# CodeKnight314/Goal-Conditioned-RL-Framework

Measured on AMD Instinct MI355X. Metric: gradient-steps/sec (HER sample + critic+actor update), higher is better.
Workload: dtype f32; 1 GPU; ddpg_pickplace_b256; agent=DDPG, batch_per_gpu=256, buffer_rows=1000000, state_dim=23, action_dim=4, hidden=256, layers=3, k_future=8, gradient_step=40, parallelism=single, hip_graph=True, rng=cpython-mt19937 (host) indices

## Files before the change

goal-conditioned-rl-framework_amd/csrc/agent_rowchain.inc:

```

struct PipeCtx {
  const StepCtrl* cur;
  const int* slot;
};


RowNet make_rownet(gcrl_agent* a, const NetSpec& n, const float* P, int which, int c = 0) {
  RowNet r;
  std::memset(&r, 0, sizeof(r));
  r.P = P;
  r.Wt = a->wt + a->wt_net[which] + (which >= 2 ? c * a->wt_cstride : 0);
  r.in = n.in_dim; r.jpad0 = round_up(n.in_dim, 4); r.H = n.H; r.L = n.L; r.out = n.out_dim;
  long long off = 0;
  for (int l = 0; l <= n.L; ++l) {
    r.w[l] = n.lin[l].w; r.b[l] = n.lin[l].b;
    if (l < n.L) { r.wt[l] = off; off += (long long)(l == 0 ? r.jpad0 : n.H) * n.H; }
  }
  return r;
}

int rc_rebuild_wt(gcrl_agent* a, hipStream_t st, bool targets_only = false) {
  auto one = [&](const RowNet& r) { return launch_wt_rebuild(st, r, const_cast<float*>(r.Wt)); };
  if (!targets_only && !a->sac) TRY(one(make_rownet(a, a->actor, a->P_actor(), 0)));
  if (a->has_target_actor) TRY(one(make_rownet(a, a->actor, a->P_tactor(), 1)));
  for (int c = 0; c < a->C; ++c) {
    if (!targets_only) TRY(one(make_rownet(a, a->critic, a->P_critic(c), 2, c)));
    TRY(one(make_rownet(a, a->critic, a->P_tcritic(c), 3, c)));
  }
  if (!targets_only) a->wt_dirty = false;
  return GCRL_OK;
}

int prof_drain(gcrl_agent* a) {
  if (a->prof_used == 0) return GCRL_OK;
  for (int i = 0; i < a->prof_used; ++i) {
    float ms = 0.f;
    GCRL_HIP(hipEventSynchronize(a->prof_b[i]));
    GCRL_HIP(hipEventElapsedTime(&ms, a->prof_a[i], a->prof_b[i]));
    a->prof_ms += ms;
  }
  std::vector<unsigned long long> clk(2 * (size_t)a->prof_used);
  GCRL_HIP(hipMemcpy(clk.data(), a->prof_clk, clk.size() * sizeof(unsigned long long), hipMemcpyDeviceToHost));
  for (int i = 0; i < a->prof_used; ++i)
    if (clk[2 * i + 1] > clk[2 * i]) a->prof_ticks += (double)(clk[2 * i + 1] - clk[2 * i]);
  a->prof_used = 0;
  return GCRL_OK;
}

bool heads_fold_on(const gcrl_agent* a) {
  return a->rowchain && a->cfg.kind == GCRL_AGENT_SAC && a->split_roles && a->slab_on() && !a->heads_fold_off && a->A <= 16 && a->bn_sync.world <= 1;
}

int rc_launch_chain(gcrl_agent* a, hipStream_t st, const PipeCtx& k, const PipeCtx& p, int what, const float* noise = nullptr) {
  RowChainArgs rc;
  std::memset(&rc, 0, sizeof(rc));
  rc.cur_k = k.cur; rc.cur_p = p.cur; rc.cb = a->ctrl();
  rc.actor = make_rownet(a, a->actor, a->P_actor(), 0);
  rc.tactor = make_rownet(a, a->actor, a->P_tactor(), 1);
  rc.C = a->C;
  for (int c = 0; c < a->C; ++c) {
    rc.critic[c] = make_rownet(a, a->critic, a->P_critic(c), 2, c);
    rc.tcritic[c] = make_rownet(a, a->critic, a->P_tcritic(c), 3, c);
  }
  const bool td3 = a->cfg.kind == GCRL_AGENT_TD3;
  rc.target_kind = a->sac ? TGT_MIN_ENT : (td3 ? TGT_MIN : TGT_DDPG);
  rc.loss_kind = td3 ? LOSS_SMOOTH_L1 : LOSS_MSE;
  if (a->sac) {
    rc.given_next = 1; rc.p_critic_only = 1;
    rc.logp_next = a->logp_next; rc.alpha = 0.2f;
    rc.pi = a->pi_buf;
  }
  rc.noise = noise; rc.policy_noise = (float)a->cfg.policy_noise; rc.noise_clamp = (float)a->cfg.noise_clamp;
  rc.seed = a->cfg.seed;
  rc.sa = a->sa; rc.nsa = a->nsa; rc.rbuf = a->rbuf; rc.dbuf = a->dbuf;
  rc.slot_x = a->slot_x; rc.slot_rd = a->slot_rd;
  rc.ldx = a->ldx; rc.ldl = a->row_ldl; rc.B = a->B; rc.S = a->S; rc.A = a->A; rc.Apad = a->Apad;
  const int nblk = (a->B + 4 * a->row_rg - 1) / (4 * a->row_rg);
  rc.linear_roles = 1;
  rc.nblk_k = (what & 1) ? nblk : 0;
  rc.nblk_p = (what & 2) ? nblk : 0;
  rc.hC = a->hC; rc.gC = a->rc_gC; rc.q = a->q; rc.y = a->ybuf; rc.dq = a->dq;
  rc.hA = a->hA; rc.gA = a->rc_gA; rc.hC2 = a->hC2; rc.q2 = a->q2; rc.dz = a->dact;
  rc.gamma = (float)a->cfg.gamma;
  rc.clamp_lo = (float)(-1.0 / (1.0 - a->cfg.gamma));
  rc.qt = a->qt;
  if (a->split_roles) {
    HeadsFold hfold;
    std::memset(&hfold, 0, sizeof(hfold));
    if (heads_fold_on(a)) {
      const NetSpec& an = a->actor;
      const long long BH = (long long)a->B * a->H;
      hfold.on = 1;
      hfold.P = a->P_actor();
      hfold.w_mean = an.lin[an.L].w; hfold.b_mean = an.lin[an.L].b; hfold.w_ls = an.lin[an.L + 1].w; hfold.b_ls = an.lin[an.L + 1].b;
      hfold.h_next = a->hN + (long long)((an.L - 1) & 1) * BH;
      hfold.h_cur = a->hA + (long long)(an.L - 1) * BH;
      hfold.eps_next = a->hf_eps_next; hfold.eps_cur = a->hf_eps_cur;
      hfold.logp_next = a->logp_next;
      hfold.pi = a->pi_buf; hfold.logp = a->logp; hfold.save_eps = a->epsbuf; hfold.save_std = a->stdbuf; hfold.head = a->headA;
      if (what & 1) {
        BnRunning& r = hfold.run;
        r.bstat[0] = a->bn_bstat; r.bstat[1] = a->hf_nf == 2 ? a->bn_bstat + (long long)an.L * 2 * a->H : nullptr;
        r.n = a->hf_nf; r.rmean = a->bn_rmean; r.rvar = a->bn_rvar; r.layers = an.L; r.H = a->H; r.B = a->B;
      }
    }
    static const bool cur_in_p = std::getenv("GCRL_HEADS_CUR_IN_P") != nullptr;
    hfold.cur_in_k = (hfold.on && a->hf_nf == 2 && !cur_in_p) ? 1 : 0;
    const HeadsFold* hfp = hfold.on ? &hfold : nullptr;
    const HeadsFold* hfp_p = (hfold.on && !hfold.cur_in_k) ? &hfold : nullptr;
    if (a->rc_merge) {
      rc.bar = reinterpret_cast<unsigned int*>(a->rc_bar); rc.status = a->status_dev;
      if (what & 1) TRY(launch_rowchain_split(st, rc, a->row_rg, 0, 3, hfp));
      if (what & 2) TRY(launch_rowchain_split(st, rc, a->row_rg, 1, 3, hfp_p));
      return GCRL_OK;
    }
    if (what & 1) { TRY(launch_rowchain_split(st, rc, a->row_rg, 0, 1, hfp)); TRY(launch_rowchain_split(st, rc, a->row_rg, 0, 2)); }
    if (what & 2) { TRY(launch_rowchain_split(st, rc, a->row_rg, 1, 1, hfp_p)); TRY(launch_rowchain_split(st, rc, a->row_rg, 1, 2)); }
    return GCRL_OK;
  }
  if (a->split_k) {
    if ((what & 1) && a->rc_merge_k) {
      rc.bar = reinterpret_cast<unsigned int*>(a->rc_bar); rc.status = a->status_dev; rc.producers_first = 1;
      TRY(launch_rowchain_split(st, rc, a->row_rg, 0, 3));
    } else if (what & 1) { TRY(launch_rowchain_split(st, rc, a->row_rg, 0, 1)); TRY(launch_rowchain_split(st, rc, a->row_rg, 0, 2)); }
    if (what & 2) { rc.nblk_k = 0; TRY(launch_rowchain_ddpg(st, rc, a->row_rg)); }
    return GCRL_OK;
  }
  if (a->ddpg_ksplit && (what & 1)) {
    rc.k_split = 1; rc.producers_first = 1;
    rc.bar = reinterpret_cast<unsigned int*>(a->rc_bar); rc.status = a->status_dev;
  }
  if (!a->prof || what != 3) return launch_rowchain_ddpg(st, rc, a->row_rg);
  if (a->prof_used == gcrl_agent::kProfPairs) TRY(prof_drain(a));
  const unsigned long long init[2] = {~0ull, 0ull};
  rc.clk = a->prof_clk + 2 * a->prof_used;
  GCRL_HIP(hipMemcpyAsync(rc.clk, init, sizeof(init), hipMemcpyHostToDevice, st));
  GCRL_HIP(hipEventRecord(a->prof_a[a->prof_used], st));
  TRY(launch_rowchain_ddpg(st, rc, a->row_rg));
  GCRL_HIP(hipEventRecord(a->prof_b[a->prof_used], st));
  a->prof_used++;
  a->prof_launches++;
  return GCRL_OK;
}

void rc_add_dw(gcrl_agent* a, Launches& ls, const PipeCtx& c, bool critic, bool fused) {
  const int B = a->B, L = a->L, H = a->H;
  const NetSpec& net = critic ? a->critic : a->actor;
  const long long BH = (long long)B * H;
  for (int k = 0; k < (critic ? a->C : 1); ++k) {
    float* Gp = critic ? a->G_critic(k) : a->G_actor();
    const float* hid = critic ? a->hC + (long long)k * L * BH : a->hA;
    const float* gr = critic ? a->rc_gC + (long long)k * L * BH : a->rc_gA;
    const float* x0 = a->sa;
    for (int l = L; l >= 0; --l) {
      const float* G = l == L ? (critic ? a->dq + (long long)k * B : a->dact) : gr + (long long)l * BH;
      const long long ldg = l == L ? (critic ? 1 : a->Apad) : H;
      GemmDesc dw = bwd_dw(G, ldg, l == 0 ? x0 : hid + (long long)(l - 1) * BH, l == 0 ? a->ldx : H, Gp, net.lin[l], B);
      if (l == 0) { dw.slot = c.slot; dw.b_slot = a->slot_x; }
      if (fused) dw.sumsq_out = critic ? a->parts_c + (long long)k * a->nparts_c + a->part_off_c[l] : a->parts_a + a->part_off_a[l];
      dw_split_form(a, dw, critic ? k : -1, l);
      ls.add(0, dw);
    }
  }
}

void rc_adam_extras(gcrl_agent* a, AdamArgs& ad, bool critic) {
  const NetSpec& net = critic ? a->critic : a->actor;
  ad.wt = a->wt + a->wt_net[critic ? 2 : 0];
  ad.wt_target = a->wt + a->wt_net[critic ? 3 : 1];
  ad.wt_net_stride = critic ? a->wt_cstride : 0;
  ad.n_seg = 0;
  int blk = 0;
  long long pos = 0, off = 0;
  auto flat = [&](long long beg, long long end) {
    if (end <= beg) return;
    AdamSeg& s = ad.seg[ad.n_seg++];
    s.beg = beg; s.dst = 0; s.rows = 1; s.cols = (int)(end - beg); s.tiled = 0; s.pad = 0;
    s.blk0 = blk; s.nblk = (int)((end - beg + 256 * kAdamPerThread - 1) / (256 * kAdamPerThread)); blk += s.nblk;
  };
  for (int l = 0; l < net.L; ++l) {
    const Lin& ln = net.lin[l];
    flat(pos, ln.w);
    AdamSeg& s = ad.seg[ad.n_seg++];
    s.beg = ln.w; s.dst = off; s.rows = ln.out; s.cols = ln.in; s.tiled = 1; s.pad = 0;
    s.blk0 = blk; s.nblk = ((ln.out + kAdamTile - 1) / kAdamTile) * ((ln.in + kAdamTile - 1) / kAdamTile); blk += s.nblk;
    pos = ln.w + (long long)ln.out * ln.in;
    off += (long long)(l == 0 ? round_up(net.in_dim, 4) : net.H) * net.H;
  }
  flat(pos, net.numel);
  ad.seg_blocks = blk;
  if (critic) {
    ad.td_q = a->q; ad.td_y = a->ybuf; ad.td_n = a->B; ad.td_C = a->C;
    ad.td_loss_kind = a->cfg.kind == GCRL_AGENT_TD3 ? LOSS_SMOOTH_L1 : LOSS_MSE;
  }
}

void of_fill_net(gcrl_agent* a, DwAdamNet& n, bool critic, int k, const StepCtrl* cur, bool polyak) {
  const int B = a->B, L = a->L, H = a->H;
  const NetSpec& net = critic ? a->critic : a->actor;
  const long long BH = (long long)B * H;
  std::memset(&n, 0, sizeof(n));
  float* Gp = critic ? a->G_critic(k) : a->G_actor();
  const float* hid = critic ? a->hC + (long long)k * L * BH : a->hA;
  const float* gr = critic ? a->rc_gC + (long long)k * L * BH : a->rc_gA;
  const std::vector<int>& poff = critic ? a->part_off_c : a->part_off_a;
  std::vector<long long> wt_off((size_t)L + 1, -1);
  long long off = 0;
  for (int l = 0; l < L; ++l) { wt_off[l] = off; off += (long long)(l == 0 ? round_up(net.in_dim, 4) : H) * H; }
  int q = 0;
  for (int l = L; l >= 0; --l, ++q) {
    const float* G = l == L ? (critic ? a->dq + (long long)k * B : a->dact) : gr + (long long)l * BH;
    const long long ldg = l == L ? (critic ? 1 : a->Apad) : H;
    GemmDesc dw = bwd_dw(G, ldg, l == 0 ? a->sa : hid + (long long)(l - 1) * BH, l == 0 ? a->ldx : H, Gp, net.lin[l], B);
    if (l == 0) { dw.slot = &cur->batch_slot; dw.b_slot = a->slot_x; }
    n.d[q] = dw;
    n.o.lay[q] = DwAdamLayer{net.lin[l].w, net.lin[l].b, wt_off[l], poff[l] / 4, 0};
  }
  n.o.nl = L + 1;
  n.o.cur = cur;
  n.o.which = critic ? 1 : 0;
  const long long go = critic ? a->goff_critic + (long long)k * a->critic_stride : a->goff_actor;
  n.o.p = critic ? a->P_critic(k) : a->P_actor();
  n.o.m = a->adam_m + go; n.o.v = a->adam_v + go;
  n.o.target = critic ? a->P_tcritic(k) : (polyak ? a->P_tactor() : nullptr);
  n.o.wt = a->wt + a->wt_net[critic ? 2 : 0] + (critic ? (long long)k * a->wt_cstride : 0);
  n.o.wt_target = a->wt + a->wt_net[critic ? 3 : 1] + (critic ? (long long)k * a->wt_cstride : 0);
  n.o.clip = (critic && k == 0 && a->cfg.kind == GCRL_AGENT_TD3) ? -1.f : (float)a->cfg.grad_clip;
  n.o.polyak = polyak ? 1 : 0;
  n.o.metric_index = critic ? MET_CRITIC_GRAD + k : MET_ACTOR_GRAD;
  const int ni = critic ? k : a->C;
  n.o.slots = reinterpret_cast<unsigned long long*>(a->of_slots) + (long long)ni * 2 * a->of_stride;
  n.o.slot_stride = (int)a->of_stride;
  n.o.seq = reinterpret_cast<unsigned int*>(a->of_seq) + ni * 32;
  if (critic) {
    if (k == 0) {
      n.o.td_q = a->q; n.o.td_y = a->ybuf; n.o.td_n = a->B; n.o.td_C = a->C;
      n.o.td_loss_kind = a->cfg.kind == GCRL_AGENT_TD3 ? LOSS_SMOOTH_L1 : LOSS_MSE;
    }
  } else {
    n.o.mean_x = a->q2; n.o.mean_n = a->B; n.o.mean_scale = -1.0f; n.o.mean_index = MET_ACTOR_LOSS;
  }
}

void of_common(gcrl_agent* a, DwAdamArgs& da) {
  std::memset(&da, 0, sizeof(da));
  da.beta2 = (float)kBeta2; da.w1 = (float)(1.0 - kBeta1); da.w2 = (float)(1.0 - kBeta2); da.eps = (float)kAdamEps;
  da.tau = (float)a->cfg.tau; da.one_m_tau = (float)(1.0 - a->cfg.tau);
  da.metrics = a->metrics_dev;
  da.status = a->status_dev;
  da.poll_first_sleep = 0; da.poll_sleep = 2; da.poll_gate = 0; da.leaders = 1;
}

bool of_phase_critics(const gcrl_agent* a, int variant) {
  return a->opt_fuse && a->cfg.kind != GCRL_AGENT_DDPG && (variant & V_FUSED_NORM) && !(variant & V_XCHG) && !(variant & V_WEIGHTS);
}
bool of_phase_actor(const gcrl_agent* a, int variant) { return of_phase_critics(a, variant) && !a->sac; }
int of_launch_critics(gcrl_agent* a, hipStream_t st, int variant) {
  DwAdamArgs da;
  of_common(a, da);
  for (int k = 0; k < a->C; ++k) of_fill_net(a, da.net[k], true, k, &a->ctrl()->cur_b, (variant & V_POLYAK_C) != 0);
  da.nnets = a->C;
  if ((variant & V_ADV) && !(variant & V_ACTOR)) da.advance = a->ctrl();
  return launch_dw_adam(st, da);
}
int of_launch_actor(gcrl_agent* a, hipStream_t st, int variant) {
  DwAdamArgs da;
  of_common(a, da);
  of_fill_net(a, da.net[0], false, 0, &a->ctrl()->cur_b, a->cfg.kind == GCRL_AGENT_TD3 && (variant & V_POLYAK_A) != 0);
  da.nnets = 1;
  if (variant & V_ADV) da.advance = a->ctrl();
  return launch_dw_adam(st, da);
}

int of_launch_ddpg(gcrl_agent* a, hipStream_t st, int what, bool adv, bool polyak) {
  DwAdamArgs da;
  of_common(a, da);
  int n = 0;
  if (what & 1) of_fill_net(a, da.net[n++], true, 0, &a->ctrl()->cur_b, polyak);
  if (what & 2) of_fill_net(a, da.net[n++], false, 0, what == 3 ? &a->ctrl()->prev_b : &a->ctrl()->cur_b, polyak);
  da.nnets = n;
  if (adv) da.advance = a->ctrl();
#ifdef GCRL_OF_STAMPS
  static unsigned long long* stamps = nullptr;
  static long long launches = 0;
  static const long long at = std::getenv("GCRL_OF_STAMPS_AT") ? std::atoll(std::getenv("GCRL_OF_STAMPS_AT")) : 3000;
  const char* path = std::getenv("GCRL_OF_STAMPS");
  if (path && !stamps) { GCRL_HIP(hipMalloc((void**)&stamps, 2 * 2048 * 8 * sizeof(unsigned long long))); }
  hipStreamCaptureStatus cs = hipStreamCaptureStatusNone;
  (void)hipStreamIsCapturing(st, &cs);
  const bool take = path && what == 3 && cs == hipStreamCaptureStatusNone && launches >= at && launches < at + 8;
  if (what == 3 && cs == hipStreamCaptureStatusNone) ++launches;
  da.stamps = take ? stamps : nullptr;
  if (take) {
    GCRL_HIP(hipMemsetAsync(stamps, 0, 2 * 2048 * 8 * sizeof(unsigned long long), st));
    TRY(launch_dw_adam(st, da));
    GCRL_HIP(hipStreamSynchronize(st));
    std::vector<unsigned long long> h(2 * 2048 * 8);
    GCRL_HIP(hipMemcpy(h.data(), stamps, h.size() * sizeof(unsigned long long), hipMemcpyDeviceToHost));
    FILE* f = std::fopen(path, launches - 1 == at ? "wb" : "ab");
    if (f) { std::fwrite(h.data(), sizeof(unsigned long long), h.size(), f); std::fclose(f); }
    return GCRL_OK;
  }
#endif
  return launch_dw_adam(st, da);
}
```

goal-conditioned-rl-framework_amd/csrc/dw_adam.h:

```cpp
#pragma once
#include "gemm_mfma.h"
#include "ops.h"

namespace gcrl {

struct DwAdamNet {
  DwAdamNetArgs o;
  GemmDesc d[kFusedMaxLayers];
};
struct DwAdamArgs {
  int nnets;
  float beta2, w1, w2, eps, tau, one_m_tau;
  float* metrics;
  CtrlBlock* advance;
  unsigned int* status;
  int leaders;
  int poll_gate;
  int poll_first_sleep, poll_sleep;
#ifdef GCRL_OF_STAMPS
  unsigned long long* stamps;
#endif
  DwAdamNet net[2];
};
int launch_dw_adam(hipStream_t st, DwAdamArgs& a);

}
```

goal-conditioned-rl-framework_amd/csrc/dw_adam.hip:

```cpp
#include "dw_adam.h"

#include <algorithm>

#include "adam_math.h"
#include "meet.h"
#include "pop.h"

namespace gcrl {
namespace {

constexpr unsigned long long kSlotEmpty = ~0ull;
constexpr int kLeaderMinTiles = 64;
static_assert(kFusedMaxLayers == 5, "DwNetHead::tile0 holds the first tiles of problems 1..4");

#ifdef GCRL_OF_STAMPS
#define OF_STAMP(k) of_t[k] = wall_clock64()
#else
#define OF_STAMP(k) do { } while (0)
#endif

template <class T>
__device__ __forceinline__ T load_uniform(const T* p) {
  static_assert(sizeof(T) % 4 == 0, "whole dwords");
  typedef const unsigned int __attribute__((address_space(4))) cu32;
  cu32* q = reinterpret_cast<cu32*>(reinterpret_cast<uintptr_t>(p));
  union { T v; unsigned int w[sizeof(T) / 4]; } u;
#pragma unroll
  for (unsigned i = 0; i < sizeof(T) / 4; ++i) u.w[i] = q[i];
  return u.v;
}

typedef float __attribute__((address_space(1))) gfloat;
typedef unsigned long long __attribute__((address_space(1))) gu64;
typedef unsigned int __attribute__((address_space(1))) gu32;

template <class T>
__device__ __forceinline__ void pin(T& v) {
  static_assert(sizeof(T) % 4 == 0, "whole dwords");
  unsigned int* w = reinterpret_cast<unsigned int*>(&v);
#pragma unroll
  for (unsigned i = 0; i < sizeof(T) / 4; ++i) asm volatile("" : "+s"(w[i]));
}

struct DwProb {
  const float* G; const float* X; float* dW; float* db;
  long long pw, pb, wt_dst;
  int ldg, ldx, out, in, K, tiles_n, slot0, x_slot;
};
struct DwNetHead {
  int ntiles, nl, which, slot_stride;
  int tile0[4];
  const StepCtrl* cur; unsigned int* seq; unsigned long long* slots;
  int polyak, grid_x;
};
struct DwNetPtrs {
  float *p, *m, *v, *target, *wt, *wt_target;
  float clip; int pad;
};
struct DwNetK {
  DwNetHead h;
  DwNetPtrs ptr;
  int metric_index, mean_n;
  const float* mean_x; float mean_scale; int mean_index;
  const float* td_q; const float* td_y; int td_n, td_C, td_loss_kind, pad;
  DwProb prob[kFusedMaxLayers];
};
struct DwAdamK {
  float beta2, w1, w2, eps, tau, one_m_tau;
  int leaders, poll_gate, poll_first_sleep, poll_sleep;
  float* metrics; CtrlBlock* advance; unsigned int* status;
#ifdef GCRL_OF_STAMPS
  unsigned long long* stamps;
#endif
  DwNetK net[2];
};

__global__ __launch_bounds__(256, 5) void dw_adam_kernel(DwAdamK a) {
  const unsigned bx = blockIdx.x, by = blockIdx.y;
#include "dw_adam_body.inc"
}

__global__ __launch_bounds__(256, 5) void dw_adam_pop_kernel(const DwAdamK* __restrict__ tab) {
  const DwAdamK& a = tab[blockIdx.z];
  const unsigned bx = blockIdx.x, by = blockIdx.y;
#include "dw_adam_body.inc"
}

}

long long dw_adam_capacity() { return meet_capacity((const void*)dw_adam_kernel, 256, 0); }

int launch_dw_adam(hipStream_t st, DwAdamArgs& a) {
  GCRL_CHECK_ARG(a.nnets >= 1 && a.nnets <= 2, "dw_adam: %d nets (1 or 2)", a.nnets);
  DwAdamK k;
  std::memset(&k, 0, sizeof(k));
  k.beta2 = a.beta2; k.w1 = a.w1; k.w2 = a.w2; k.eps = a.eps; k.tau = a.tau; k.one_m_tau = a.one_m_tau;
  k.leaders = a.leaders; k.poll_gate = a.poll_gate; k.poll_first_sleep = a.poll_first_sleep; k.poll_sleep = a.poll_sleep;
  k.metrics = a.metrics; k.advance = a.advance; k.status = a.status;
#ifdef GCRL_OF_STAMPS
  k.stamps = a.stamps;
#endif
  int widest = 0;
  for (int i = 0; i < a.nnets; ++i) {
    DwAdamNet& n = a.net[i];
    DwNetK& kn = k.net[i];
    GCRL_CHECK_ARG(n.o.nl >= 1 && n.o.nl <= kFusedMaxLayers && n.o.slots && n.o.seq && n.o.cur, "dw_adam: net %d: %d problems / missing slots", i, n.o.nl);
    int tiles = 0;
    for (int l = 0; l < n.o.nl; ++l) {
      GemmDesc& d = n.d[l];
      GCRL_CHECK_ARG(d.M >= 1 && d.N >= 2 && d.K >= 1 && d.A && d.B && d.C && d.ones_col && d.col_out && !d.bias && d.epi == EPI_NONE && d.mul == MUL_NONE &&
                         !d.bn_part && d.ksplit <= 1 && d.shape_hint == 0 && gemm_shape_of(d) == 1,
                     "dw_adam: net %d problem %d is not a dW | db problem of the k-split 16x16 form", i, l);
      GCRL_CHECK_ARG(d.a_rs == 1 && d.b_cs == 1 && d.c_rs == d.N - 1 && d.a_cs < (1LL << 31) && d.b_rs < (1LL << 31) && d.a_slot == 0 && d.c_slot == 0 &&
                         (!d.slot || (d.slot == &n.o.cur->batch_slot && d.b_slot < (1LL << 31))),
                     "dw_adam: net %d problem %d is not laid out like a dW | db problem", i, l);
      DwProb& p = kn.prob[l];
      p.G = d.A; p.X = d.B; p.dW = d.C; p.db = d.col_out;
      p.pw = n.o.lay[l].pw; p.pb = n.o.lay[l].pb; p.wt_dst = n.o.lay[l].wt_dst;
      p.ldg = (int)d.a_cs; p.ldx = (int)d.b_rs; p.out = d.M; p.in = d.N - 1; p.K = d.K;
      p.tiles_n = (d.N + 15) / 16; p.slot0 = n.o.lay[l].slot0; p.x_slot = d.slot ? (int)d.b_slot : 0;
      if (l >= 1) kn.h.tile0[l - 1] = tiles;
      tiles += ((d.M + 15) / 16) * p.tiles_n;
    }
    n.o.ntiles = tiles;
    GCRL_CHECK_ARG(tiles <= 256 * kFusedMaxSlotsPerThread && tiles + 8 <= n.o.slot_stride, "dw_adam: net %d has %d tiles (slots: %d)", i, tiles, n.o.slot_stride);
    widest = std::max(widest, tiles);
    for (int l = n.o.nl; l < kFusedMaxLayers; ++l) kn.h.tile0[l - 1] = 0x7fffffff;
    kn.h.ntiles = tiles; kn.h.nl = n.o.nl; kn.h.which = n.o.which; kn.h.slot_stride = n.o.slot_stride;
    kn.h.cur = n.o.cur; kn.h.seq = n.o.seq; kn.h.slots = n.o.slots;
    kn.ptr.p = n.o.p; kn.ptr.m = n.o.m; kn.ptr.v = n.o.v; kn.ptr.target = n.o.target; kn.ptr.wt = n.o.wt; kn.ptr.wt_target = n.o.wt_target;
    kn.ptr.clip = n.o.clip; kn.h.polyak = n.o.polyak; kn.metric_index = n.o.metric_index;
    kn.mean_x = n.o.mean_x; kn.mean_n = n.o.mean_n; kn.mean_scale = n.o.mean_scale; kn.mean_index = n.o.mean_index;
    kn.td_q = n.o.td_q; kn.td_y = n.o.td_y; kn.td_n = n.o.td_n; kn.td_C = n.o.td_C; kn.td_loss_kind = n.o.td_loss_kind;
  }
  for (int i = 0; i < a.nnets; ++i) k.net[i].h.grid_x = widest;
  if (PopRec* r = pop_recording())
    return pop_record(r, POP_DW_ADAM, 0, dim3((unsigned)widest, (unsigned)a.nnets), 0, &k, sizeof(k), [k, g = dim3((unsigned)widest, (unsigned)a.nnets)](hipStream_t s) -> int {
      hipLaunchKernelGGL(dw_adam_kernel, g, dim3(256), 0, s, k);
      GCRL_HIP(hipGetLastError());
      return GCRL_OK;
    });
  hipLaunchKernelGGL(dw_adam_kernel, dim3((unsigned)widest, (unsigned)a.nnets), dim3(256), 0, st, k);
  GCRL_HIP(hipGetLastError());
  return GCRL_OK;
}

long long dw_adam_pop_capacity() { return meet_capacity((const void*)dw_adam_pop_kernel, 256, 0); }

int launch_dw_adam_pop(hipStream_t st, const void* tab, int members, dim3 grid) {
  GCRL_CHECK_ARG(members >= 1 && members <= 65535 && grid.y >= 1 && grid.y <= 2 && grid.z == 1, "dw_adam population: bad launch");
  hipLaunchKernelGGL(dw_adam_pop_kernel, dim3(grid.x, grid.y, (unsigned)members), dim3(256), 0, st, static_cast<const DwAdamK*>(tab));
  GCRL_HIP(hipGetLastError());
  return GCRL_OK;
}

}
```

goal-conditioned-rl-framework_amd/csrc/dw_adam_body.inc:

```
#ifdef GCRL_OF_STAMPS
  unsigned long long of_t[5];
#endif
  OF_STAMP(0);
  __shared__ float s_ss[4];
  __shared__ double dred[4];
  __shared__ float s_coef;
  __shared__ float tile_p[16][17], tile_t[16][17];
  const DwNetK& on = a.net[by];
  DwNetHead o = on.h;
  pin(o);
  if ((int)bx >= o.ntiles) return;
  const unsigned long long t_start = wall_clock64();
  int bid = (int)bx;
  {
    const int per = o.ntiles >> 3;
    if (bid < (per << 3)) bid = ((bid + (int)by * o.grid_x) & 7) * per + (bid >> 3);
  }
  const int lane = threadIdx.x & 63;
  const int wave = __builtin_amdgcn_readfirstlane(threadIdx.x >> 6);
  const int li = lane & 15, lg = lane >> 4;
  const int pi = (bid >= o.tile0[0]) + (bid >= o.tile0[1]) + (bid >= o.tile0[2]) + (bid >= o.tile0[3]);
  const int t0 = pi == 0 ? 0 : o.tile0[0] * (pi == 1) + o.tile0[1] * (pi == 2) + o.tile0[2] * (pi == 3) + o.tile0[3] * (pi == 4);
  DwProb pr = on.prob[pi];
  DwNetPtrs ptr = on.ptr;
  StepCtrl c = load_uniform(o.cur);
  unsigned long long sq = load_uniform(reinterpret_cast<const unsigned long long*>(o.seq));
  pin(pr); pin(ptr); pin(c); pin(sq);
  gfloat* const gp = (gfloat*)ptr.p; gfloat* const gm = (gfloat*)ptr.m; gfloat* const gv = (gfloat*)ptr.v; gfloat* const gt = (gfloat*)ptr.target;
  gfloat* const gwt = (gfloat*)ptr.wt; gfloat* const gwtt = (gfloat*)ptr.wt_target;
  gu64* const gslots = (gu64*)o.slots;
  const unsigned int seq = (unsigned int)sq, fault = (unsigned int)(sq >> 32);
  const int t = bid - t0;
  const int tn = t % pr.tiles_n, tm = t / pr.tiles_n;
  const int m0 = tm << 4, n0 = tn << 4;
  const int in = pr.in, out = pr.out;
  struct { long long pw, pb, wt_dst; int slot0; } lay = {pr.pw, pr.pb, pr.wt_dst, pr.slot0};

  const AdamStepScalars sc = adam_scalars(c, o.which);
  const int em = m0 + 4 * lg + wave, en = n0 + li;
  long long my_i = -1;
  if (em < out) {
    if (en < in) my_i = lay.pw + (long long)em * in + en;
    else if (en == in) my_i = lay.pb + em;
  }
  const bool pk = ptr.target && o.polyak;

  GemmDesc d;
  d.A = pr.G; d.a_rs = 1; d.a_cs = pr.ldg;
  d.B = pr.X + (pr.x_slot ? (long long)c.batch_slot * pr.x_slot : 0); d.b_rs = pr.ldx; d.b_cs = 1;
  int one = 1;
  asm volatile("" : "+s"(one));
  d.C = pr.dW; d.c_rs = pr.in; d.col_out = pr.db; d.ones_col = one;
  d.M = pr.out; d.N = pr.in + 1; d.K = pr.K;
  d.bias = nullptr; d.H = nullptr; d.h_rs = 0; d.epi = EPI_NONE; d.mul = MUL_NONE;
  d.slot = nullptr; d.a_slot = d.b_slot = d.c_slot = d.h_slot = 0;
  d.sumsq_out = nullptr; d.bn_part = nullptr;
  d.a_vec = d.b_vec = d.a_rvec = d.b_rvec = 0;
  d.tile0 = 0; d.tiles_n = pr.tiles_n; d.ntiles = 0x7fffffff;
  d.shape_hint = 0; d.ksplit = 0; d.kpart = nullptr; d.kticket = nullptr;
  float x, ss;
  OF_STAMP(1);
  gemm_batch_tile<1, 1, 4>(d, t, x, ss);

#pragma unroll
  for (int off = 32; off > 0; off >>= 1) ss += __shfl_down(ss, off, 64);
  if (lane == 0) s_ss[wave] = ss;
  __syncthreads();
  gu64* mine = gslots + (long long)(seq & 1u) * o.slot_stride;
  if (threadIdx.x == 0 && !(fault && bid == 1)) {
    const double dt = ((double)s_ss[0] + (double)s_ss[1]) + ((double)s_ss[2] + (double)s_ss[3]);
    const int slot = lay.slot0 + t;
    __hip_atomic_store(mine + slot, (unsigned long long)__double_as_longlong(dt), __ATOMIC_RELAXED, __HIP_MEMORY_SCOPE_AGENT);
    gslots[(long long)((seq & 1u) ^ 1u) * o.slot_stride + slot] = kSlotEmpty;
  }
  float pre_p = 0.f, pre_m = 0.f, pre_v = 0.f, pre_t = 0.f;
  if (my_i >= 0) {
    pre_p = gp[my_i]; pre_m = gm[my_i]; pre_v = gv[my_i];
    if (pk) pre_t = gt[my_i];
  }
  OF_STAMP(2);
  float* met = a.metrics + (long long)c.metrics_slot * kMetricFloats;
  if (bid == 0) {
    if (on.mean_x) rider_mean_metric(on.mean_x, on.mean_n, on.mean_scale, met + on.mean_index);
    if (on.td_q) rider_td_metrics(on.td_q, on.td_y, on.td_n, on.td_C, on.td_loss_kind, met);
  }
  {
    const bool lead_mode = a.leaders && o.ntiles >= kLeaderMinTiles;
    const bool sweeper = !lead_mode || bx < 8;
    const int xc = ((int)bx + (int)by * o.grid_x) & 7;
    gu64* res = mine + (o.slot_stride - 8);
    bool ok = true;
    double s = 0.0;
    if (sweeper) {
      unsigned long long w[kFusedMaxSlotsPerThread];
      int spins = 0;
      for (int i = 0; i < a.poll_first_sleep; ++i) __builtin_amdgcn_s_sleep(1);
      for (int i = 0; i < 4096 && (long long)(wall_clock64() - t_start) < (long long)a.poll_gate; ++i) __builtin_amdgcn_s_sleep(2);
#pragma unroll
      for (int u = 0; u < kFusedMaxSlotsPerThread; ++u) {
        const int i = (int)threadIdx.x + 256 * u;
        w[u] = i < o.ntiles ? __hip_atomic_load(mine + i, __ATOMIC_RELAXED, __HIP_MEMORY_SCOPE_AGENT) : 0ull;
      }
      for (;;) {
        bool all = true;
#pragma unroll
        for (int u = 0; u < kFusedMaxSlotsPerThread; ++u) all = all && w[u] != kSlotEmpty;
        if (all) break;
        if (++spins >= kMeetSpinMax) { ok = false; break; }
        for (int i = 0; i < a.poll_sleep; ++i) __builtin_amdgcn_s_sleep(1);
#pragma unroll
        for (int u = 0; u < kFusedMaxSlotsPerThread; ++u)
          if (w[u] == kSlotEmpty) w[u] = __hip_atomic_load(mine + (int)threadIdx.x + 256 * u, __ATOMIC_RELAXED, __HIP_MEMORY_SCOPE_AGENT);
      }
#pragma unroll
      for (int u = 0; u < kFusedMaxSlotsPerThread; ++u)
        if ((int)threadIdx.x + 256 * u < o.ntiles) s += __longlong_as_double((long long)w[u]);
      if (!ok) s = __longlong_as_double(0x7ff8000000000000ll);
      s = wave_sum_d(s);
      if (lane == 0) dred[wave] = s;
      __syncthreads();
      if (threadIdx.x == 0) {
        s = dred[0] + dred[1] + dred[2] + dred[3];
        if (lead_mode) {
          __hip_atomic_store(res + xc, (unsigned long long)__double_as_longlong(s), __ATOMIC_RELAXED, __HIP_MEMORY_SCOPE_AGENT);
          gslots[(long long)((seq & 1u) ^ 1u) * o.slot_stride + (o.slot_stride - 8) + xc] = kSlotEmpty;
        }
      }
    } else if (threadIdx.x == 0) {
      unsigned long long w = __hip_atomic_load(res + xc, __ATOMIC_RELAXED, __HIP_MEMORY_SCOPE_AGENT);
      for (int spins = 0; w == kSlotEmpty; ) {
        if (++spins >= kMeetSpinMax) { ok = false; w = 0x7ff8000000000000ull; break; }
        for (int i = 0; i < a.poll_sleep; ++i) __builtin_amdgcn_s_sleep(1);
        w = __hip_atomic_load(res + xc, __ATOMIC_RELAXED, __HIP_MEMORY_SCOPE_AGENT);
      }
      s = __longlong_as_double((long long)w);
    }
    if (!ok && a.status) __hip_atomic_fetch_or(a.status, (unsigned int)MEET_ERR_DW_ADAM, __ATOMIC_RELAXED, __HIP_MEMORY_SCOPE_SYSTEM);
    if (threadIdx.x == 0) {
      float post;
      s_coef = clip_coef(s, c.grad_scale, ptr.clip, &post);
      if (bid == 0 && a.metrics) met[on.metric_index] = post;
    }
  }
  __syncthreads();
  OF_STAMP(3);
  const float gmul = c.grad_scale * s_coef;
  float p_new = 0.f, t_new = 0.f;
  if (my_i >= 0) {
    const AdamElem e = adam_elem(x, pre_p, pre_m, pre_v, gmul, sc, a.beta2, a.w1, a.w2, a.eps);
    gp[my_i] = e.p; gm[my_i] = e.m; gv[my_i] = e.v;
    p_new = e.p;
    if (pk) { t_new = polyak_elem(a.tau, e.p, a.one_m_tau, pre_t); gt[my_i] = t_new; }
  }
  if (lay.wt_dst >= 0) {
    tile_p[4 * lg + wave][li] = p_new;
    tile_t[4 * lg + wave][li] = t_new;
    __syncthreads();
    const int ty = threadIdx.x >> 4, tx = threadIdx.x & 15;
    const int k = n0 + ty, oo = m0 + tx;
    if (k < in && oo < out) {
      const long long at = lay.wt_dst + (long long)k * out + oo;
      gwt[at] = tile_p[tx][ty];
      if (pk && ptr.wt_target) gwtt[at] = tile_t[tx][ty];
    }
  }
  OF_STAMP(4);
#ifdef GCRL_OF_STAMPS
  if (a.stamps && threadIdx.x == 0)
    for (int k = 0; k < 5; ++k) a.stamps[((long long)by * 2048 + bx) * 8 + k] = of_t[k];
#endif
  if (bid == 0 && threadIdx.x == 0) {
    ((gu32*)o.seq)[1] = 0u;
    ((gu32*)o.seq)[0] = seq + 1u;
    if (by == 0 && a.advance) ctrl_advance(a.advance);
  }
```

Before: 19430 gradient-steps/s.

## Stage Adam state tiles through LDS with 128-bit buffer loads and stores

For full, aligned 16x16 tiles, each wave loads one of the p/m/v/target arrays as a 16x16 tile with 128-bit buffer loads issued before the grad-norm meet, stages it in shared memory, runs Adam/Polyak from LDS, and writes back with wide stores, including the transposed Wt copy. This aims to replace scattered per-element global accesses with coalesced vector traffic and to hide the load latency behind the global reduction wait. Irregular tiles keep the old path. It also removes the runtime poll tunables (leaders, gate, sleep counts) and hardcodes the same defaults, at the cost of an extra LDS buffer and a barrier.

```diff
diff --git a/goal-conditioned-rl-framework_amd/csrc/agent_rowchain.inc b/goal-conditioned-rl-framework_amd/csrc/agent_rowchain.inc
--- a/goal-conditioned-rl-framework_amd/csrc/agent_rowchain.inc
+++ b/goal-conditioned-rl-framework_amd/csrc/agent_rowchain.inc
@@ -248,7 +248,6 @@
   da.tau = (float)a->cfg.tau; da.one_m_tau = (float)(1.0 - a->cfg.tau);
   da.metrics = a->metrics_dev;
   da.status = a->status_dev;
-  da.poll_first_sleep = 0; da.poll_sleep = 2; da.poll_gate = 0; da.leaders = 1;
 }
 
 bool of_phase_critics(const gcrl_agent* a, int variant) {
diff --git a/goal-conditioned-rl-framework_amd/csrc/dw_adam.h b/goal-conditioned-rl-framework_amd/csrc/dw_adam.h
--- a/goal-conditioned-rl-framework_amd/csrc/dw_adam.h
+++ b/goal-conditioned-rl-framework_amd/csrc/dw_adam.h
@@ -14,9 +14,6 @@
   float* metrics;
   CtrlBlock* advance;
   unsigned int* status;
-  int leaders;
-  int poll_gate;
-  int poll_first_sleep, poll_sleep;
 #ifdef GCRL_OF_STAMPS
   unsigned long long* stamps;
 #endif
diff --git a/goal-conditioned-rl-framework_amd/csrc/dw_adam.hip b/goal-conditioned-rl-framework_amd/csrc/dw_adam.hip
--- a/goal-conditioned-rl-framework_amd/csrc/dw_adam.hip
+++ b/goal-conditioned-rl-framework_amd/csrc/dw_adam.hip
@@ -11,6 +11,8 @@
 
 constexpr unsigned long long kSlotEmpty = ~0ull;
 constexpr int kLeaderMinTiles = 64;
+constexpr int kSc1 = 16;
+constexpr int kImgLd = 20;
 static_assert(kFusedMaxLayers == 5, "DwNetHead::tile0 holds the first tiles of problems 1..4");
 
 #ifdef GCRL_OF_STAMPS
@@ -33,6 +35,11 @@
 typedef float __attribute__((address_space(1))) gfloat;
 typedef unsigned long long __attribute__((address_space(1))) gu64;
 typedef unsigned int __attribute__((address_space(1))) gu32;
+
+__device__ __forceinline__ void poll_pause() {
+  __builtin_amdgcn_s_sleep(1);
+  __builtin_amdgcn_s_sleep(1);
+}
 
 template <class T>
 __device__ __forceinline__ void pin(T& v) {
@@ -67,7 +74,6 @@
 };
 struct DwAdamK {
   float beta2, w1, w2, eps, tau, one_m_tau;
-  int leaders, poll_gate, poll_first_sleep, poll_sleep;
   float* metrics; CtrlBlock* advance; unsigned int* status;
 #ifdef GCRL_OF_STAMPS
   unsigned long long* stamps;
@@ -95,7 +101,6 @@
   DwAdamK k;
   std::memset(&k, 0, sizeof(k));
   k.beta2 = a.beta2; k.w1 = a.w1; k.w2 = a.w2; k.eps = a.eps; k.tau = a.tau; k.one_m_tau = a.one_m_tau;
-  k.leaders = a.leaders; k.poll_gate = a.poll_gate; k.poll_first_sleep = a.poll_first_sleep; k.poll_sleep = a.poll_sleep;
   k.metrics = a.metrics; k.advance = a.advance; k.status = a.status;
 #ifdef GCRL_OF_STAMPS
   k.stamps = a.stamps;
diff --git a/goal-conditioned-rl-framework_amd/csrc/dw_adam_body.inc b/goal-conditioned-rl-framework_amd/csrc/dw_adam_body.inc
--- a/goal-conditioned-rl-framework_amd/csrc/dw_adam_body.inc
+++ b/goal-conditioned-rl-framework_amd/csrc/dw_adam_body.inc
@@ -6,11 +6,11 @@
   __shared__ double dred[4];
   __shared__ float s_coef;
   __shared__ float tile_p[16][17], tile_t[16][17];
+  __shared__ __attribute__((aligned(16))) float img[4][16][kImgLd];
   const DwNetK& on = a.net[by];
   DwNetHead o = on.h;
   pin(o);
   if ((int)bx >= o.ntiles) return;
-  const unsigned long long t_start = wall_clock64();
   int bid = (int)bx;
   {
     const int per = o.ntiles >> 3;
@@ -73,8 +73,19 @@
     __hip_atomic_store(mine + slot, (unsigned long long)__double_as_longlong(dt), __ATOMIC_RELAXED, __HIP_MEMORY_SCOPE_AGENT);
     gslots[(long long)((seq & 1u) ^ 1u) * o.slot_stride + slot] = kSlotEmpty;
   }
+  int in_q = in, out_q = out;
+  asm volatile("" : "+s"(in_q), "+s"(out_q) :: "memory");
+  const bool wt_wide = lay.wt_dst < 0 || ((out_q & 3) == 0 && (lay.wt_dst & 3) == 0 &&
+                                          (((unsigned long long)ptr.wt | (pk ? (unsigned long long)ptr.wt_target : 0ull)) & 15) == 0);
+  const bool regular = (in_q & 3) == 0 && n0 + 16 <= in_q && m0 + 16 <= out_q && (lay.pw & 3) == 0 && wt_wide &&
+                       (((unsigned long long)ptr.p | (unsigned long long)ptr.m | (unsigned long long)ptr.v | (pk ? (unsigned long long)ptr.target : 0ull)) & 15) == 0;
+  const bool mover = wave < 3 || pk;
+  const int r4 = lane >> 2, c4 = (lane & 3) << 2;
+  const float* const my_arr = wave == 0 ? ptr.p : wave == 1 ? ptr.m : wave == 2 ? ptr.v : ptr.target;
   float pre_p = 0.f, pre_m = 0.f, pre_v = 0.f, pre_t = 0.f;
-  if (my_i >= 0) {
+  v4u pre4 = {0u, 0u, 0u, 0u};
+  if (regular && mover) pre4 = __builtin_amdgcn_raw_buffer_load_b128(wave_uniform_rsrc_n(my_arr + lay.pw + (long long)m0 * in + n0, 15LL * in + 16), (r4 * in + c4) * 4, 0, 0);
+  if (!regular && my_i >= 0) {
     pre_p = gp[my_i]; pre_m = gm[my_i]; pre_v = gv[my_i];
     if (pk) pre_t = gt[my_i];
   }
@@ -85,7 +96,7 @@
     if (on.td_q) rider_td_metrics(on.td_q, on.td_y, on.td_n, on.td_C, on.td_loss_kind, met);
   }
   {
-    const bool lead_mode = a.leaders && o.ntiles >= kLeaderMinTiles;
+    const bool lead_mode = o.ntiles >= kLeaderMinTiles;
     const bool sweeper = !lead_mode || bx < 8;
     const int xc = ((int)bx + (int)by * o.grid_x) & 7;
     gu64* res = mine + (o.slot_stride - 8);
@@ -94,8 +105,6 @@
     if (sweeper) {
       unsigned long long w[kFusedMaxSlotsPerThread];
       int spins = 0;
-      for (int i = 0; i < a.poll_first_sleep; ++i) __builtin_amdgcn_s_sleep(1);
-      for (int i = 0; i < 4096 && (long long)(wall_clock64() - t_start) < (long long)a.poll_gate; ++i) __builtin_amdgcn_s_sleep(2);
 #pragma unroll
       for (int u = 0; u < kFusedMaxSlotsPerThread; ++u) {
         const int i = (int)threadIdx.x + 256 * u;
@@ -107,7 +116,7 @@
         for (int u = 0; u < kFusedMaxSlotsPerThread; ++u) all = all && w[u] != kSlotEmpty;
         if (all) break;
         if (++spins >= kMeetSpinMax) { ok = false; break; }
-        for (int i = 0; i < a.poll_sleep; ++i) __builtin_amdgcn_s_sleep(1);
+        poll_pause();
 #pragma unroll
         for (int u = 0; u < kFusedMaxSlotsPerThread; ++u)
           if (w[u] == kSlotEmpty) w[u] = __hip_atomic_load(mine + (int)threadIdx.x + 256 * u, __ATOMIC_RELAXED, __HIP_MEMORY_SCOPE_AGENT);
@@ -130,7 +139,7 @@
       unsigned long long w = __hip_atomic_load(res + xc, __ATOMIC_RELAXED, __HIP_MEMORY_SCOPE_AGENT);
       for (int spins = 0; w == kSlotEmpty; ) {
         if (++spins >= kMeetSpinMax) { ok = false; w = 0x7ff8000000000000ull; break; }
-        for (int i = 0; i < a.poll_sleep; ++i) __builtin_amdgcn_s_sleep(1);
+        poll_pause();
         w = __hip_atomic_load(res + xc, __ATOMIC_RELAXED, __HIP_MEMORY_SCOPE_AGENT);
       }
       s = __longlong_as_double((long long)w);
@@ -142,17 +151,34 @@
       if (bid == 0 && a.metrics) met[on.metric_index] = post;
     }
   }
+  if (regular && mover) *reinterpret_cast<v4u*>(&img[wave][r4][c4]) = pre4;
   __syncthreads();
   OF_STAMP(3);
   const float gmul = c.grad_scale * s_coef;
   float p_new = 0.f, t_new = 0.f;
-  if (my_i >= 0) {
+  if (regular) {
+    const int r = 4 * lg + wave;
+    const AdamElem e = adam_elem(x, img[0][r][li], img[1][r][li], img[2][r][li], gmul, sc, a.beta2, a.w1, a.w2, a.eps);
+    if (pk) img[3][r][li] = polyak_elem(a.tau, e.p, a.one_m_tau, img[3][r][li]);
+    img[0][r][li] = e.p; img[1][r][li] = e.m; img[2][r][li] = e.v;
+    __syncthreads();
+    if (mover)
+      __builtin_amdgcn_raw_buffer_store_b128(*reinterpret_cast<const v4u*>(&img[wave][r4][c4]), wave_uniform_rsrc_n(my_arr + lay.pw + (long long)m0 * in + n0, 15LL * in + 16),
+                                             (r4 * in + c4) * 4, 0, kSc1);
+    const bool cp_t = wave == 2 && pk && ptr.wt_target;
+    if (lay.wt_dst >= 0 && (wave == 3 || cp_t)) {
+      const float (*src)[kImgLd] = cp_t ? img[3] : img[0];
+      const v4u run = {__float_as_uint(src[c4][r4]), __float_as_uint(src[c4 + 1][r4]), __float_as_uint(src[c4 + 2][r4]), __float_as_uint(src[c4 + 3][r4])};
+      __builtin_amdgcn_raw_buffer_store_b128(run, wave_uniform_rsrc_n((cp_t ? ptr.wt_target : ptr.wt) + lay.wt_dst + (long long)n0 * out + m0, 15LL * out + 16),
+                                             (r4 * out + c4) * 4, 0, kSc1);
+    }
+  } else if (my_i >= 0) {
     const AdamElem e = adam_elem(x, pre_p, pre_m, pre_v, gmul, sc, a.beta2, a.w1, a.w2, a.eps);
     gp[my_i] = e.p; gm[my_i] = e.m; gv[my_i] = e.v;
     p_new = e.p;
     if (pk) { t_new = polyak_elem(a.tau, e.p, a.one_m_tau, pre_t); gt[my_i] = t_new; }
   }
-  if (lay.wt_dst >= 0) {
+  if (!regular && lay.wt_dst >= 0) {
     tile_p[4 * lg + wave][li] = p_new;
     tile_t[4 * lg + wave][li] = t_new;
     __syncthreads();
```

Measured after the change: 19650 gradient-steps/s (median of 6 runs). 1.01x the previous value.
